# DanEngelbrecht/longtail

Measured on AMD Instinct MI355X. Metric: ingest GB/s (chunk+hash+compress), higher is better.
Workload: dtype u8/u32

## Files before the change

longtail_amd/csrc/k_buzhash.hip:

```cpp
#include "lthip_internal.h"

#include <stdlib.h>
#include <type_traits>

namespace
{

__constant__ uint32_t c_buztab[256] = {
#include "buzhash_table.inc"
};

constexpr int RUN = 64;
constexpr int TILE = 256 * RUN;
constexpr int ROW_DW = 17;
constexpr int TAB_REP = 64;

__device__ __forceinline__ uint32_t lds_load_u32(uint32_t byte_addr)
{
#if defined(__HIP_DEVICE_COMPILE__)
    return *(const __attribute__((address_space(3))) uint32_t*)byte_addr;
#else
    (void)byte_addr;
    return 0u;
#endif
// ... 139 lines not shown
    auto group = [&](auto G) __attribute__((always_inline))
    {
        constexpr int g = decltype(G)::value;
        uint32_t y[8];
#pragma unroll
        for (int half = 1; half >= 0; --half)
        {
            if (half == 1)
                halo_wait(std::integral_constant<int, 2 * g + 1 + 4>{});
            else
                halo_wait(std::integral_constant<int, 2 * g + 4>{});
#pragma unroll
            for (int ii = 3; ii >= 0; --ii)
            {
                const int i = 4 * half + ii;
                const int k = 8 * g + i;
                uint32_t w;
                if (k >= 47)
                    w = S[k - 47] ^ S[k + 1];
                else
                    w = (S[0] ^ S[k + 1]) ^ (uint32_t)__builtin_amdgcn_update_dpp(0, (int)S[(k + 17) & 63], 0x13C, 0xf, 0xf, false);
                const uint32_t h = (k & 31) ? rotl32(w, (uint32_t)(k & 31)) : w;
                if (MODE == 1)
                    y[i] = ~h & (dv.d - 1u);
                else
                {
#if K1_MAD64
                    uint64_t t, carry;
                    asm("v_mad_u64_u32 %0, %1, %2, %3, %4" : "=v"(t), "=s"(carry) : "v"(h), "s"(dv.inv), "v"(inv64));
                    y[i] = (uint32_t)t;
#else
                    y[i] = h * dv.inv + inv_v;
#endif
                }
            }
            if (half == 1)
                halo_quad(std::integral_constant<int, 2 * g + 2>{});
            else
                halo_quad(std::integral_constant<int, 2 * g + 1>{});
        }
        const uint32_t m = min(min(min(y[0], y[1]), y[2]), min(min(min(y[3], y[4]), y[5]), min(y[6], y[7])));
        if (__builtin_amdgcn_ballot_w64(m <= pc.thr) != 0ull)
        {
            asm volatile("");
#pragma unroll
            for (int i = 0; i < 8; ++i)
            {
                const int k = 8 * g + i;
                if (__builtin_amdgcn_ballot_w64(y[i] <= pc.thr) != 0ull)
                {
                    asm volatile("");
                    const bool hit = MODE == 1 ? y[i] == 0u : rotr32(y[i] + pc.exact_add, dv.k2) <= dv.qlim;
                    uint32_t hbit;
                    asm volatile("v_cndmask_b32_e64 %0, 0, 1, %1" : "=v"(hbit) : "s"(__builtin_amdgcn_ballot_w64(hit)));
                    if (k < 32)
                        mlo |= hbit << k;
                    else
                        mhi |= hbit << (k - 32);
                }
            }
        }
    };
    group(std::integral_constant<int, 7>{});
    group(std::integral_constant<int, 6>{});
    group(std::integral_constant<int, 5>{});
    group(std::integral_constant<int, 4>{});
    group(std::integral_constant<int, 3>{});
    group(std::integral_constant<int, 2>{});
    group(std::integral_constant<int, 1>{});
    group(std::integral_constant<int, 0>{});
    return ((uint64_t)mhi << 32) | mlo;
}

__device__ __forceinline__ uint64_t prefix_legal(uint64_t m, uint64_t q0, uint64_t size)
{
    if (q0 >= size)
        return 0ull;
    if (q0 < 47)
        m &= ~0ull << (47 - q0);
    const uint64_t remain = size - q0;
    if (remain < 64)
        m &= (1ull << remain) - 1ull;
    return m;
}

__device__ __forceinline__ void prefix_table_init(uint32_t* tab, int tid, int nthreads)
{
    for (int v = tid; v < 256; v += nthreads)
    {
        const uint32_t tv = c_buztab[v];
        uint4 q = make_uint4(tv, tv, tv, tv);
        uint4* dst = reinterpret_cast<uint4*>(tab + v * TAB_REP);
#pragma unroll
        for (int j = 0; j < TAB_REP / 4; ++j)
            dst[j] = q;
    }
    __syncthreads();
    if ((uint32_t)(uintptr_t)(const __attribute__((address_space(3))) uint32_t*)tab != 0u)
        __builtin_trap();
}

#ifdef LTHIP_ABLATIONS
#include "ablations/k_buzhash_prefix_regs.inc"
#endif

constexpr int DMA_BUF_B = WROWS * 64;

struct TileDma
{
    const uint8_t* data;
    uint32_t* buf;
    int lane;
    uint32_t buf_byte;
    uint32_t buf_mid;
    uint32_t src_off;
    uint32_t own_row;
    uint32_t own_f;

    __device__ __forceinline__ TileDma(const uint8_t* d, uint32_t* b, int ln) : data(d), buf(b), lane(ln)
    {
        buf_byte = __builtin_amdgcn_readfirstlane((uint32_t)(uintptr_t)(const __attribute__((address_space(3))) uint32_t*)buf);
        buf_mid = buf_byte + 2048u;
        const uint32_t src_vec = 4u * ((uint32_t)lane >> 2) + (((uint32_t)lane & 3u) ^ (((uint32_t)lane >> 4) & 3u));
        src_off = 16u * src_vec;
        own_f = (((uint32_t)lane + 1u) >> 2) & 3u;
        own_row = buf_byte + 64u * ((uint32_t)lane + 1u);
    }

    template <int MODE>
    __device__ __forceinline__ PrefixConsts consts(const DivTest& dv) const
    {
        PrefixConsts pc;
        pc.lane4 = (uint32_t)lane * 4u;
        pc.hj = 63u - (uint32_t)lane;
        pc.halo_byte = buf_byte + DMA_BUF_B;
        pc.thr = MODE == 1 ? 0u : 0xFFFFFFFFu / (dv.d >> dv.k2);
        pc.exact_add = dv.addc - dv.inv;
        return pc;
    }

    template <int u>
    __device__ __forceinline__ void piece(const uint8_t* mid_src) const
    {
        asm volatile("s_mov_b32 m0, %[l]\n\ts_nop 0\n\t"
                     "global_load_lds_dwordx4 %[v], %[b] offset:%[o]"
                     :
                     : [v] "v"(src_off), [l] "s"(buf_mid), [b] "s"(mid_src), [o] "i"(1024 * u - 2048)
                     : "memory");
    }

    template <int u>
    __device__ __forceinline__ void edge(const PartDev& p, uint64_t sp, const uint8_t* mid_src) const
    {
        const int64_t g = (int64_t)sp - 64 + 1024 * u + (int64_t)src_off;
        const bool lane_on = u < 4 || lane < 4;
        const bool whole = lane_on && g >= 0 && (uint64_t)g + 16 <= p.size;
        const bool part = lane_on && g >= 0 && (uint64_t)g < p.size && (uint64_t)g + 16 > p.size;
        if (whole)
            piece<u>(mid_src);
        if (part)
        {
            const uint8_t* src = data + p.off;
            uint32_t w[4] = {0, 0, 0, 0};
            const uint32_t n = (uint32_t)(p.size - (uint64_t)g);
            for (uint32_t bb = 0; bb < n; ++bb)
                w[bb >> 2] |= (uint32_t)src[g + bb] << (8 * (bb & 3));
            uint32_t* d = buf + 256 * u + 4 * lane;
            d[0] = w[0];
            d[1] = w[1];
            d[2] = w[2];
            d[3] = w[3];
        }
    }

    __device__ __forceinline__ void issue(const PartDev& p, uint64_t sp) const
    {
        const uint8_t* mid_src = data + p.off + sp - 64 + 2048;
        if (sp >= 64 && sp + (uint64_t)WTILE <= p.size)
        {
            asm volatile("s_mov_b32 m0, %[l]\n\ts_nop 0\n\t"
                         "global_load_lds_dwordx4 %[v], %[b] offset:-2048\n\t"
                         "global_load_lds_dwordx4 %[v], %[b] offset:-1024\n\t"
                         "global_load_lds_dwordx4 %[v], %[b] offset:0\n\t"
                         "global_load_lds_dwordx4 %[v], %[b] offset:1024"
                         :
                         : [v] "v"(src_off), [l] "s"(buf_mid), [b] "s"(mid_src)
                         : "memory");
            if (lane < 4)
                piece<4>(mid_src);
        }
        else
        {
            edge<0>(p, sp, mid_src);
            edge<1>(p, sp, mid_src);
            edge<2>(p, sp, mid_src);
            edge<3>(p, sp, mid_src);
            edge<4>(p, sp, mid_src);
        }
    }

    __device__ __forceinline__ void take(uint32_t (&win)[16], uint32_t& hb, const PrefixConsts& pc) const
    {
        asm volatile("s_waitcnt vmcnt(0)" ::: "memory");
#pragma unroll
        for (int c = 0; c < 4; ++c)
        {
            const uint4 q = lds_load_u128(own_row + 16u * ((uint32_t)c ^ own_f));
            win[4 * c + 0] = q.x;
            win[4 * c + 1] = q.y;
            win[4 * c + 2] = q.z;
            win[4 * c + 3] = q.w;
        }
        hb = lds_load_u8(buf_byte + pc.hj);
        asm volatile("s_waitcnt lgkmcnt(0)" ::: "memory");
    }
};

template <int MODE, int WAVES>
__global__ __launch_bounds__(64 * WAVES, 1) void k_buzhash_prefix_dma(const uint8_t* __restrict__ data,
                                                                       const PartDev* __restrict__ parts,
                                                                       const uint32_t* __restrict__ tile_part,
                                                                       uint32_t ntiles, DivTest dv,
                                                                       uint64_t* __restrict__ bm0,
                                                                       uint64_t* __restrict__ bm1)
{
    extern __shared__ __attribute__((aligned(16))) uint32_t smem[];
    const int tid = threadIdx.x;
    const int lane = tid & 63;
    const int wave = __builtin_amdgcn_readfirstlane(tid >> 6);
    uint32_t* buf = smem + 256 * TAB_REP + wave * ((DMA_BUF_B >> 2) + HALO_DW);
    uint32_t* halo = buf + (DMA_BUF_B >> 2);
    prefix_table_init(smem, tid, 64 * WAVES);

    const TileDma dma(data, buf, lane);
    const PrefixConsts pc = dma.consts<MODE>(dv);

    const uint64_t nwt = (uint64_t)ntiles * 4u;
    const uint64_t wstride = (uint64_t)gridDim.x * (uint64_t)WAVES;
    uint64_t wt = (uint64_t)blockIdx.x * (uint64_t)WAVES + (uint64_t)wave;
    if (wt >= nwt)
        return;

    PartDev pd = parts[tile_part[wt >> 2]];
    uint64_t span = ((wt >> 2) - pd.tile_base) * (uint64_t)TILE + (wt & 3u) * (uint64_t)WTILE;
    dma.issue(pd, span);

    uint64_t pend_m = 0, pend_summary = 0, pend_i0 = 0, pend_i1 = 0;
    bool pend = false;
    for (;;)
    {
        uint32_t win[16], hb;
        dma.take(win, hb, pc);

        if (pend)
        {
            if (pend_m != 0ull)
                bm0[pend_i0 + (uint64_t)lane] = pend_m;
            if (lane == 0)
                bm1[pend_i1] = pend_summary;
        }

        const uint64_t next = wt + wstride;
        PartDev npd = pd;
        uint64_t next_span = 0;
        if (next < nwt)
        {
            npd = parts[tile_part[next >> 2]];
            next_span = ((next >> 2) - npd.tile_base) * (uint64_t)TILE + (next & 3u) * (uint64_t)WTILE;
            dma.issue(npd, next_span);
        }

        pend_m = prefix_legal(prefix_tile<MODE>(win, hb, pc, dv, lane, halo), span + (uint64_t)lane * RUN, pd.size);
        pend_summary = __builtin_amdgcn_ballot_w64(pend_m != 0ull);
        pend_i0 = pd.bm0_base + (span >> 6);
        pend_i1 = pd.bm1_base + (span >> 12);
        pend = true;

        if (next >= nwt)
            break;
        wt = next;
        pd = npd;
        span = next_span;
    }
    if (pend_m != 0ull)
        bm0[pend_i0 + (uint64_t)lane] = pend_m;
    if (lane == 0)
        bm1[pend_i1] = pend_summary;
}

__device__ __forceinline__ uint64_t bcast64(uint64_t v, int src_lane)
{
    uint32_t lo = __builtin_amdgcn_readlane((uint32_t)v, src_lane);
    uint32_t hi = __builtin_amdgcn_readlane((uint32_t)(v >> 32), src_lane);
    return ((uint64_t)hi << 32) | lo;
}

__global__ __launch_bounds__(64) void k_select_cuts(const PartDev* __restrict__ parts, uint32_t nparts,
                                                    const uint64_t* __restrict__ bm0, const uint64_t* __restrict__ bm1,
                                                    uint32_t min_chunk, uint32_t max_chunk, uint2* __restrict__ region,
                                                    uint32_t* __restrict__ part_count)
{
    const uint32_t p = blockIdx.x;
    if (p >= nparts)
        return;
    const int lane = threadIdx.x;
    const PartDev pd = parts[p];
    const uint64_t size = pd.size;
    const uint64_t* b0 = bm0 + pd.bm0_base;
    const uint64_t* b1 = bm1 + pd.bm1_base;
    uint2* out = region + pd.region_base;

    uint64_t s = 0;
    uint32_t n = 0;
    while (s < size)
    {
        const uint64_t left = size - s;
        uint64_t len;
        if (left <= min_chunk)
            len = left;
        else
        {
            const uint64_t end = left > max_chunk ? max_chunk : left;
            len = end;
            const uint64_t qlo = s + min_chunk;
            const uint64_t qhi = s + end - 1;
            if (qlo <= qhi)
            {
                const uint64_t rlo = qlo >> 6, rhi = qhi >> 6;
                const uint64_t wlo = rlo >> 6, whi = rhi >> 6;
                bool found = false;
                for (uint64_t w0 = wlo; w0 <= whi && !found; w0 += 64)
                {
                    const uint64_t w = w0 + (uint64_t)lane;
                    uint64_t word = 0;
                    if (w <= whi)
                    {
                        word = b1[w];
                        if (w == wlo)
                            word &= ~0ull << (rlo & 63);
                        if (w == whi && (rhi & 63) != 63)
                            word &= (1ull << ((rhi & 63) + 1)) - 1ull;
                    }
                    for (;;)
                    {
                        const uint64_t any = __builtin_amdgcn_ballot_w64(word != 0ull);
                        if (any == 0ull)
                            break;
                        const int f = __builtin_ctzll(any);
                        const uint64_t fw = bcast64(word, f);
                        const int bit = __builtin_ctzll(fw);
                        const uint64_t r = ((w0 + (uint64_t)f) << 6) + (uint64_t)bit;
                        uint64_t m = b0[r];
                        if (r == rlo)
                            m &= ~0ull << (qlo & 63);
                        if (r == rhi && (qhi & 63) != 63)
                            m &= (1ull << ((qhi & 63) + 1)) - 1ull;
                        if (m != 0ull)
                        {
                            const uint64_t q = (r << 6) + (uint64_t)__builtin_ctzll(m);
                            len = q - s + 1;
                            found = true;
                            break;
                        }
                        if (lane == f)
                            word &= word - 1ull;
                    }
                }
            }
        }
        if (lane == 0)
            out[n] = make_uint2((uint32_t)s, (uint32_t)len);
        ++n;
        s += len;
    }
    if (lane == 0)
        part_count[p] = n;
}

#ifdef LTHIP_ABLATIONS
__device__ unsigned long long g_walk_tiles;
#endif

template <int MODE, int WAVES, bool GUESS>
__global__ __launch_bounds__(64 * WAVES, 1) void k_buzhash_walk(const uint8_t* __restrict__ data, const PartDev* __restrict__ parts,
                                                                 uint32_t nparts, DivTest dv, uint32_t min_chunk, uint32_t max_chunk,
                                                                 uint2* __restrict__ region, uint32_t* __restrict__ part_count,
                                                                 uint32_t* __restrict__ ticket)
{
    extern __shared__ __attribute__((aligned(16))) uint32_t smem[];
    const int tid = threadIdx.x;
    const int lane = tid & 63;
    const int wave = __builtin_amdgcn_readfirstlane(tid >> 6);
    uint32_t* buf = smem + 256 * TAB_REP + wave * ((DMA_BUF_B >> 2) + HALO_DW);
    uint32_t* halo = buf + (DMA_BUF_B >> 2);
    prefix_table_init(smem, tid, 64 * WAVES);

    const TileDma dma(data, buf, lane);
    const PrefixConsts pc = dma.consts<MODE>(dv);
    const int lane_base = lane * RUN;

    auto jump = [](uint64_t q) __attribute__((always_inline)) { return q >= 64 ? ((q - 64) & ~(uint64_t)15) + 64 : (uint64_t)0; };

    bool inflight = false;
    uint64_t inflight_tb = 0;
#ifdef LTHIP_ABLATIONS
    uint32_t tiles = 0;
#endif
    for (;;)
    {
        __builtin_amdgcn_wave_barrier();
        uint32_t t = atomicAdd(ticket, lane == 0 ? 1u : 0u);
        t = __builtin_amdgcn_readfirstlane(t);
        if (t >= nparts)
            break;
        const PartDev pd = parts[t];
        const uint64_t size = pd.size;
        uint2* out = region + pd.region_base;
        uint64_t s = 0, qlo = 0, qhi = 0;
        uint32_t n = 0, end = 0;

        auto next_chunk = [&]() __attribute__((always_inline)) -> bool
        {
            for (;;)
            {
                if (s >= size)
                    return false;
                const uint64_t left = size - s;
                const uint32_t len = left <= min_chunk ? (uint32_t)left : left > max_chunk ? max_chunk : (uint32_t)left;
                if (left > min_chunk && len > min_chunk)
                {
                    end = len;
                    qlo = s + min_chunk;
                    qhi = s + end - 1;
                    return true;
                }
                if (lane == 0)
                    out[n] = make_uint2((uint32_t)s, len);
                ++n;
                s += len;
            }
        };

        if (next_chunk())
        {
            uint64_t tb = jump(qlo);
            for (bool walking = true; walking;)
            {
                if (!(inflight && inflight_tb == tb))
                {
                    if (inflight)
                        asm volatile("s_waitcnt vmcnt(0)" ::: "memory");
                    dma.issue(pd, tb);
                }
                inflight = false;
                uint32_t win[16], hb;
                dma.take(win, hb, pc);
                if (GUESS)
                {
                    uint64_t g = tb + (uint64_t)WTILE;
                    bool aim = true;
                    if (g > qhi)
                    {
                        const uint64_t s2 = s + end;
                        aim = size - s2 > min_chunk && max_chunk > min_chunk;
                        g = jump(s2 + min_chunk);
                    }
                    if (aim)
                    {
                        dma.issue(pd, g);
                        inflight = true;
                        inflight_tb = g;
                    }
                }
                const uint64_t raw = prefix_tile<MODE>(win, hb, pc, dv, lane, halo);
#ifdef LTHIP_ABLATIONS
                ++tiles;
#endif
                for (;;)
                {
                    const int lo = (int)(qlo > tb ? qlo - tb : 0) - lane_base;
                    const int hi = (int)(qhi - tb < (uint64_t)WTILE ? qhi - tb : (uint64_t)WTILE - 1) - lane_base;
                    uint64_t m = raw;
                    if (lo > 0)
                        m = lo > 63 ? 0ull : m & (~0ull << lo);
                    if (hi < 63)
                        m = hi < 0 ? 0ull : m & ((2ull << hi) - 1ull);
                    const uint64_t any = __builtin_amdgcn_ballot_w64(m != 0ull);
                    uint32_t len;
                    if (any != 0ull)
                    {
                        const int f = __builtin_ctzll(any);
                        const uint64_t q = tb + (uint64_t)(f * RUN + __builtin_ctzll(bcast64(m, f)));
                        len = (uint32_t)(q - s) + 1u;
                    }
                    else if (qhi - tb < (uint64_t)WTILE)
                        len = end;
                    else
                    {
                        tb += (uint64_t)WTILE;
                        break;
                    }
                    if (lane == 0)
                        out[n] = make_uint2((uint32_t)s, len);
                    ++n;
                    s += len;
                    if (!next_chunk())
                    {
                        walking = false;
                        break;
                    }
                    if (qlo >= tb && qlo - tb < (uint64_t)WTILE)
                        continue;
                    tb = jump(qlo);
                    break;
                }
            }
        }
        if (inflight)
        {
            asm volatile("s_waitcnt vmcnt(0)" ::: "memory");
            inflight = false;
        }
        if (lane == 0)
            part_count[t] = n;
    }
#ifdef LTHIP_ABLATIONS
    if (lane == 0 && tiles)
        atomicAdd(&g_walk_tiles, (unsigned long long)tiles);
#endif
}

constexpr int SCAN_THREADS = 256;
constexpr int SCAN_ITEMS = 8;
constexpr int SCAN_BLOCK = SCAN_THREADS * SCAN_ITEMS;

__device__ __forceinline__ uint32_t block_exclusive_scan(uint32_t v, uint32_t* total, uint32_t* sh )
{
    const int lane = threadIdx.x & 63, wave = threadIdx.x >> 6;
    uint32_t x = v;
#pragma unroll
    for (int o = 1; o < 64; o <<= 1)
    {
        uint32_t y = __shfl_up(x, o, 64);
        if (lane >= o)
            x += y;
    }
    if (lane == 63)
        sh[wave] = x;
    __syncthreads();
    uint32_t base = 0, tot = 0;
#pragma unroll
    for (int w = 0; w < SCAN_THREADS / 64; ++w)
    {
        uint32_t t = sh[w];
        if (w < wave)
            base += t;
        tot += t;
    }
    __syncthreads();
    *total = tot;
    return base + x - v;
}

__global__ __launch_bounds__(SCAN_THREADS) void k_scan_sums(const uint32_t* __restrict__ in, uint64_t n,
                                                            const uint32_t* __restrict__ n_dev,
                                                            uint32_t* __restrict__ sums)
{
    __shared__ uint32_t sh[8];
    if (n_dev)
        n = *n_dev < n ? *n_dev : n;
    const uint64_t base = (uint64_t)blockIdx.x * SCAN_BLOCK;
    uint32_t acc = 0;
#pragma unroll
    for (int i = 0; i < SCAN_ITEMS; ++i)
    {
        uint64_t idx = base + (uint64_t)i * SCAN_THREADS + threadIdx.x;
        if (idx < n)
            acc += in[idx];
    }
    uint32_t tot;
    block_exclusive_scan(acc, &tot, sh);
    if (threadIdx.x == 0)
        sums[blockIdx.x] = tot;
}

__global__ __launch_bounds__(SCAN_THREADS) void k_scan_spine(uint32_t* __restrict__ sums, uint32_t nblocks)
{
    __shared__ uint32_t sh[8];
    uint32_t carry = 0;
    for (uint32_t b0 = 0; b0 < nblocks; b0 += SCAN_THREADS)
    {
        uint32_t i = b0 + threadIdx.x;
        uint32_t v = i < nblocks ? sums[i] : 0;
        uint32_t tot;
        uint32_t ex = block_exclusive_scan(v, &tot, sh);
        if (i < nblocks)
            sums[i] = carry + ex;
        carry += tot;
    }
    if (threadIdx.x == 0)
        sums[nblocks] = carry;
}

__global__ __launch_bounds__(SCAN_THREADS) void k_scan_apply(const uint32_t* __restrict__ in, uint64_t n,
                                                             const uint32_t* __restrict__ n_dev,
                                                             const uint32_t* __restrict__ sums, uint32_t nblocks,
                                                             uint32_t* __restrict__ out)
{
    __shared__ uint32_t sh[8];
    if (n_dev)
        n = *n_dev < n ? *n_dev : n;
    const uint64_t base = (uint64_t)blockIdx.x * SCAN_BLOCK + (uint64_t)threadIdx.x * SCAN_ITEMS;
    uint32_t v[SCAN_ITEMS];
    uint32_t acc = 0;
#pragma unroll
    for (int i = 0; i < SCAN_ITEMS; ++i)
    {
        uint64_t idx = base + i;
        v[i] = idx < n ? in[idx] : 0;
        acc += v[i];
    }
    uint32_t tot;
    uint32_t ex = block_exclusive_scan(acc, &tot, sh) + sums[blockIdx.x];
#pragma unroll
    for (int i = 0; i < SCAN_ITEMS; ++i)
    {
        uint64_t idx = base + i;
        if (idx < n)
            out[idx] = ex;
        ex += v[i];
    }
    if (blockIdx.x == 0 && threadIdx.x == 0)
        out[n] = sums[nblocks];
}

__global__ __launch_bounds__(64) void k_compact_chunks(const PartDev* __restrict__ parts, uint32_t nparts,
                                                       const uint2* __restrict__ region,
                                                       const uint32_t* __restrict__ part_first,
                                                       uint64_t* __restrict__ chunk_offsets,
                                                       uint32_t* __restrict__ chunk_lens)
{
    const uint32_t p = blockIdx.x;
    if (p >= nparts)
        return;
    const PartDev pd = parts[p];
    const uint32_t first = part_first[p];
    const uint32_t n = part_first[p + 1] - first;
    const uint2* in = region + pd.region_base;
    for (uint32_t i = threadIdx.x; i < n; i += 64)
    {
        uint2 e = in[i];
        chunk_offsets[first + i] = pd.off + (uint64_t)e.x;
        chunk_lens[first + i] = e.y;
    }
}

__global__ __launch_bounds__(64) void k_chunk_from_buffer(const uint8_t* __restrict__ buf, uint32_t n, uint32_t min_chunk,
                                                          DivTest dv, uint64_t* __restrict__ out_len)
{
    const int lane = threadIdx.x;
    uint32_t h0 = 0;
    for (uint32_t i = 0; i < 48; ++i)
        h0 ^= rotl32(c_buztab[buf[i]], (47u - i) & 31u);
    uint32_t result = n;
// ... 278 lines not shown
```

longtail_amd/csrc/lthip_ctx.hip:

```cpp
#include "lthip_internal.h"

#include <stdlib.h>

int lthip_fail(lthip_ctx* ctx, int code, const char* what, const char* detail)
{
    if (ctx)
        snprintf(ctx->err, sizeof ctx->err, "%s: %s", what ? what : "?", detail ? detail : "");
    return code;
}

int lthip_scratch(lthip_ctx* ctx, int slot, size_t bytes, void** out)
{
    if (bytes == 0)
        bytes = 256;
    if (ctx->scratch_cap[slot] < bytes)
    {
        if (ctx->scratch[slot])
        {
            LTHIP_CHECK(ctx, lthip_stream_wait(ctx));
            LTHIP_CHECK(ctx, hipFree(ctx->scratch[slot]));
            ctx->scratch[slot] = nullptr;
            ctx->scratch_cap[slot] = 0;
        }
        size_t cap = bytes + bytes / 8 + 4096;
// ... 509 lines not shown
    block_starts[nb] = i;
    *out_block_count = nb;
    *out_next_chunk = i;
    return 0;
}

extern "C" int lthip_divtest_eval(uint32_t discriminator, uint32_t hash)
{
    if (discriminator == 0)
        return 0;
    const DivTest t = make_div_test(discriminator);
    if (t.pow2)
        return (hash & (t.d - 1u)) == t.d - 1u;
    const uint32_t m = hash * t.inv + t.addc;
    const uint32_t r = t.k2 ? ((m >> t.k2) | (m << (32u - t.k2))) : m;
    return r <= t.qlim;
}

static uint32_t plan_slice_points(uint32_t part_count, const uint64_t* part_sizes, uint32_t want, uint32_t* first)
{
    if (part_count < 2 || want < 2)
        return 0;
    uint64_t total = 0;
    for (uint32_t p = 0; p < part_count; ++p)
        total += part_sizes[p];
    if (total < LTHIP_SLICE_MIN_BYTES)
        return 0;
    uint32_t S = want > part_count ? part_count : want;
    while (S > 2 && total / S < LTHIP_SLICE_MIN_BYTES / 2)
        --S;
    uint64_t acc = 0;
    uint32_t p = 0;
    first[0] = 0;
    for (uint32_t k = 1; k < S; ++k)
    {
        const uint64_t goal = total / S * k;
        while (p < part_count - (S - k) && acc + part_sizes[p] / 2 < goal)
            acc += part_sizes[p++];
        if (p <= first[k - 1])
        {
            acc += part_sizes[p];
            ++p;
        }
        first[k] = p;
    }
    first[S] = part_count;
    return S;
}

static int plan_layout(lthip_ctx* ctx, const char* what, uint32_t min_chunk, uint32_t part_count, const uint64_t* part_offsets,
                       const uint64_t* part_sizes, PartDev* parts, PlanExtents& x)
{
    memset(&x, 0, sizeof x);
    x.nparts = part_count;
    for (uint32_t p = 0; p < part_count; ++p)
    {
        const uint64_t sz = part_sizes[p];
        if ((part_offsets[p] & 15u) != 0 || sz > 0xFFFFFFFFull)
            return lthip_fail(ctx, EINVAL, what, "part offsets must be 16-byte aligned, sizes < 4 GiB");
        PartDev& pd = parts[p];
        memset(&pd, 0, sizeof pd);
        pd.off = part_offsets[p];
        pd.size = sz;
        pd.bm0_base = x.bm0_words;
        pd.bm1_base = x.bm1_words;
        pd.region_base = x.chunk_cap;
        pd.tile_base = (uint32_t)x.ntiles;
        const uint64_t cap = sz ? sz / min_chunk + 1 : 0;
        pd.region_cap = (uint32_t)cap;
        const uint64_t t = div_up_u64(sz, 16384);
        x.ntiles += t;
        x.bm0_words += t * 256;
        x.bm1_words += t * 4;
        x.chunk_cap += cap;
        x.total_bytes += sz;
        x.leaf_cap += div_up_u64(sz, 1024) + cap;
        x.nonempty_parts += sz != 0;
        x.max_part_bytes = sz > x.max_part_bytes ? sz : x.max_part_bytes;
    }
    return 0;
}

static bool plan_walk_rule(const lthip_plan* plan)
{
    const uint64_t waves = lthip_k1_resident_waves(plan->device);
    return plan->nonempty_parts >= LTHIP_WALK_MIN_PARTS_PER_WAVE * waves &&
           plan->max_part_bytes * LTHIP_WALK_MAX_PART_DIV <= plan->total_bytes / waves;
}

static int plan_create_impl(lthip_ctx* ctx, uint32_t part_count, const uint64_t* part_offsets, const uint64_t* part_sizes,
                            uint32_t min_chunk, uint32_t avg_chunk, uint32_t max_chunk, lthip_plan** out_plan)
{
    if (!ctx || !out_plan || (part_count && (!part_offsets || !part_sizes)))
        return EINVAL;
    *out_plan = nullptr;
    if (min_chunk < 48 || min_chunk > avg_chunk || avg_chunk > max_chunk)
        return lthip_fail(ctx, EINVAL, "lthip_plan_create", "need 48 <= min <= avg <= max");
    uint32_t d = discriminator_from_avg(avg_chunk);
    if (d == 0)
        return lthip_fail(ctx, EINVAL, "lthip_plan_create", "discriminator is zero");
    LTHIP_CHECK(ctx, hipSetDevice(ctx->device));
    std::vector<PartDev> parts(part_count);
    PlanExtents x;
    int err = plan_layout(ctx, "lthip_plan_create", min_chunk, part_count, part_offsets, part_sizes, parts.data(), x);
    if (err)
        return err;
    if (x.ntiles > 0xFFFFFFF0ull)
        return lthip_fail(ctx, EINVAL, "lthip_plan_create", "batch too large");

    lthip_plan* plan = new (std::nothrow) lthip_plan();
    if (!plan)
        return ENOMEM;
    memset(plan, 0, sizeof *plan);
    static_cast<PlanExtents&>(*plan) = x;
    plan->device = ctx->device;
    plan->min_chunk = min_chunk;
    plan->avg_chunk = avg_chunk;
    plan->max_chunk = max_chunk;
    plan->div = make_div_test(d);
    plan->capacity_bytes = x.total_bytes;
    plan->cap_parts = part_count ? part_count : 1;
    plan->cap_tiles = x.ntiles ? x.ntiles : 1;
    plan->walked = plan_walk_rule(plan);

    hipError_t e = lthip_hip_malloc((void**)&plan->d_parts, sizeof(PartDev) * plan->cap_parts);
    if (e == hipSuccess)
        e = lthip_hip_malloc((void**)&plan->d_tile_part, sizeof(uint32_t) * plan->cap_tiles);
    if (e == hipSuccess && part_count)
        e = hipMemcpyAsync(plan->d_parts, parts.data(), sizeof(PartDev) * part_count, hipMemcpyHostToDevice, ctx->stream);
    if (e == hipSuccess)
        e = lthip_stream_wait(ctx);
    if (e != hipSuccess)
    {
        lthip_plan_destroy(ctx, plan);
        return lthip_fail(ctx, e == hipErrorOutOfMemory ? ENOMEM : EIO, "lthip_plan_create", hipGetErrorString(e));
    }
    if ((err = lthip_launch_tile_table(ctx, plan)))
    {
        lthip_plan_destroy(ctx, plan);
        return err;
    }
    *out_plan = plan;
    return 0;
}

static int plan_aim(lthip_ctx* ctx, lthip_plan* plan, const PlanExtents& x, const PartDev* parts)
{
    static_cast<PlanExtents&>(*plan) = x;
    plan->walked = plan_walk_rule(plan);
    const int err = lthip_stage_upload(ctx, plan->d_parts, parts, sizeof(PartDev) * x.nparts, ctx->stream);
    return err ? err : lthip_launch_tile_table(ctx, plan);
}

static void plan_aim_slices(lthip_ctx* ctx, lthip_plan* plan, uint32_t want, const uint64_t* part_offsets, const uint64_t* part_sizes)
{
    plan->sliced = false;
    uint32_t first[9];
    const uint32_t S = plan_slice_points(plan->nparts, part_sizes, want, first);
    if (S == 0 || (plan->nslices && S != plan->nslices))
        return;
    bool ok = true;
    if (!plan->nslices)
        for (uint32_t k = 0; k < S && ok; ++k)
            ok = plan_create_impl(ctx, first[k + 1] - first[k], part_offsets + first[k], part_sizes + first[k], plan->min_chunk,
                                  plan->avg_chunk, plan->max_chunk, &plan->slice[k]) == 0;
    else
    {
        std::vector<PartDev> parts(plan->nparts);
        PlanExtents x[8];
        for (uint32_t k = 0; k < S && ok; ++k)
        {
            const uint32_t n = first[k + 1] - first[k];
            ok = plan_layout(ctx, "lthip_plan_reaim", plan->min_chunk, n, part_offsets + first[k], part_sizes + first[k], &parts[first[k]],
                             x[k]) == 0 &&
                 n <= plan->slice[k]->cap_parts && x[k].ntiles <= plan->slice[k]->cap_tiles;
        }
        for (uint32_t k = 0; k < S && ok; ++k)
            ok = plan_aim(ctx, plan->slice[k], x[k], &parts[first[k]]) == 0;
    }
    if (!ok)
    {
        if (!plan->nslices)
            for (uint32_t k = 0; k < S; ++k)
            {
                lthip_plan_destroy(ctx, plan->slice[k]);
                plan->slice[k] = nullptr;
            }
        ctx->err[0] = 0;
        return;
    }
    memcpy(plan->slice_first, first, sizeof(uint32_t) * (S + 1));
    plan->nslices = S;
    plan->sliced = true;
}

extern "C" int lthip_plan_create(lthip_ctx* ctx, uint32_t part_count, const uint64_t* part_offsets,
                                 const uint64_t* part_sizes, uint32_t min_chunk, uint32_t avg_chunk, uint32_t max_chunk,
                                 lthip_plan** out_plan)
{
    int err = plan_create_impl(ctx, part_count, part_offsets, part_sizes, min_chunk, avg_chunk, max_chunk, out_plan);
    if (err)
        return err;
    int want = LTHIP_SLICES;
    LTHIP_ABLATION_ENV(env_slices, "LTHIP_SLICES");
    if (env_slices.get() > 0)
        want = env_slices.get() > 8 ? 8 : env_slices.get();
    plan_aim_slices(ctx, *out_plan, (uint32_t)want, part_offsets, part_sizes);
    return 0;
}

extern "C" int lthip_plan_resize_single(lthip_ctx* ctx, lthip_plan* plan, uint64_t size)
{
    if (!ctx || !plan || plan->nparts != 1)
        return EINVAL;
    if (size > plan->capacity_bytes)
        return lthip_fail(ctx, EINVAL, "lthip_plan_resize_single", "size above the capacity the plan was created with");
    LTHIP_CHECK(ctx, hipSetDevice(ctx->device));
    const uint64_t off = 0;
    PartDev pd;
    PlanExtents x;
    const int err = plan_layout(ctx, "lthip_plan_resize_single", plan->min_chunk, 1, &off, &size, &pd, x);
    if (err)
        return err;
    static_cast<PlanExtents&>(*plan) = x;
    return lthip_stage_upload(ctx, plan->d_parts, &pd, sizeof pd, ctx->stream);
}

extern "C" int lthip_plan_reaim(lthip_ctx* ctx, lthip_plan* plan, uint32_t part_count, const uint64_t* part_offsets,
                                const uint64_t* part_sizes)
{
    if (!ctx || !plan || (part_count && (!part_offsets || !part_sizes)))
        return EINVAL;
    if (part_count == 0 || part_count > plan->cap_parts)
        return lthip_fail(ctx, EINVAL, "lthip_plan_reaim", "part count outside 1 .. the count the plan was created with");
    LTHIP_CHECK(ctx, hipSetDevice(ctx->device));
    {
        std::vector<PartDev> parts(part_count);
        PlanExtents x;
        int err = plan_layout(ctx, "lthip_plan_reaim", plan->min_chunk, part_count, part_offsets, part_sizes, parts.data(), x);
        if (err)
            return err;
        if (x.ntiles > plan->cap_tiles)
            return lthip_fail(ctx, EINVAL, "lthip_plan_reaim", "more 16 KiB tiles than the plan was created with");
        if ((err = plan_aim(ctx, plan, x, parts.data())))
            return err;
    }
    if (plan->nslices)
        plan_aim_slices(ctx, plan, plan->nslices, part_offsets, part_sizes);
    return 0;
}

extern "C" void lthip_plan_destroy(lthip_ctx* ctx, lthip_plan* plan)
{
    if (!plan)
        return;
    (void)hipSetDevice(plan->device);
    if (ctx)
        (void)lthip_stream_wait(ctx);
    else
        (void)hipDeviceSynchronize();
    if (plan->d_parts)
        (void)hipFree(plan->d_parts);
    if (plan->d_tile_part)
        (void)hipFree(plan->d_tile_part);
    for (uint32_t k = 0; k < 8; ++k)
        lthip_plan_destroy(ctx, plan->slice[k]);
    delete plan;
}

extern "C" uint64_t lthip_plan_chunk_capacity(const lthip_plan* plan) { return plan ? plan->chunk_cap : 0; }
extern "C" uint32_t lthip_plan_slices(const lthip_plan* plan) { return plan && plan->sliced ? plan->nslices : 1u; }

static bool plan_walks(const lthip_plan* plan)
{
    LTHIP_ABLATION_ENV(env_walk, "LTHIP_K1_WALK");
    if (env_walk.get() >= 0)
        return env_walk.get() != 0 && plan->nparts != 0;
    return plan->walked;
}
extern "C" uint32_t lthip_plan_walked_scans(const lthip_plan* plan)
{
    if (!plan)
        return 0;
    if (!plan->sliced)
        return plan_walks(plan);
    uint32_t n = 0;
    for (uint32_t k = 0; k < plan->nslices; ++k)
        n += plan_walks(plan->slice[k]);
    return n;
}

struct ScanBuffers
{
    uint64_t *bm0, *bm1;
    uint2* region;
    uint32_t* part_count;
};
static int chunk_scan_buffers(lthip_ctx* ctx, const lthip_plan* plan, bool bitmaps, ScanBuffers* b)
{
    b->bm0 = b->bm1 = nullptr;
    int err;
    if (bitmaps && ((err = lthip_scratch(ctx, S_BM0, plan->bm0_words * 8, (void**)&b->bm0)) ||
                    (err = lthip_scratch(ctx, S_BM1, plan->bm1_words * 8, (void**)&b->bm1))))
        return err;
    if ((err = lthip_scratch(ctx, S_REGION, plan->chunk_cap * sizeof(uint2), (void**)&b->region)))
        return err;
    return lthip_scratch(ctx, S_PART_COUNT, ((size_t)plan->nparts + 1) * 4, (void**)&b->part_count);
}

static int chunk_scan(lthip_ctx* ctx, const lthip_plan* plan, const void* d_data, const ScanBuffers& b)
{
    if (!plan->nparts)
        return 0;
    return plan_walks(plan) ? lthip_launch_buzhash_walk(ctx, plan, (const uint8_t*)d_data, b.region, b.part_count)
                            : lthip_launch_buzhash(ctx, plan, (const uint8_t*)d_data, b.bm0, b.bm1);
}

static int chunk_cut_hash(lthip_ctx* ctx, const lthip_plan* plan, const void* d_data, const ScanBuffers& b, uint64_t* d_offsets,
                          uint32_t* d_lens, uint64_t* d_hashes, uint32_t* d_part_first)
{
    int err;
    if (plan->nparts && !plan_walks(plan) && (err = lthip_launch_select(ctx, plan, b.bm0, b.bm1, b.region, b.part_count)))
        return err;
    if ((err = lthip_launch_compact(ctx, plan, b.region, b.part_count, d_part_first, d_offsets, d_lens)))
        return err;
    return d_hashes ? lthip_launch_blake3(ctx, (const uint8_t*)d_data, d_offsets, d_lens, d_part_first + plan->nparts, plan->chunk_cap,
                                          plan->leaf_cap, plan->max_chunk, d_hashes)
                    : 0;
}

__global__ void k_slice_join(const uint64_t* __restrict__ b_off, const uint32_t* __restrict__ b_len, const uint64_t* __restrict__ b_hash,
                             const uint32_t* __restrict__ b_first, uint32_t nparts_b, uint32_t* __restrict__ part_first ,
                             uint64_t* __restrict__ offs, uint32_t* __restrict__ lens, uint64_t* __restrict__ hashes)
{
    const uint32_t base = part_first[0], total_b = b_first[nparts_b];
    const uint64_t i = (uint64_t)blockIdx.x * blockDim.x + threadIdx.x;
    if (i < total_b)
    {
        offs[base + i] = b_off[i];
        lens[base + i] = b_len[i];
        hashes[base + i] = b_hash[i];
    }
    if (i >= 1 && i <= nparts_b)
        part_first[i] = b_first[i] + base;
}

// ... 141 lines not shown
```

Baseline: 903.4.

## Simplify edge/bound arithmetic to 32-bit and skip slicing for walking plans

Edge handling in the buzhash DMA tile loader now computes the valid byte window per 1 KiB piece with 32-bit comparisons. It reads partial tails relative to the mid source pointer instead of doing 64-bit per-lane bounds checks. The bitmap store base is forced into scalar registers, and the cut-walk range tests use unsigned 32-bit wraparound compares. On the host, plans that use the walk rule no longer run in sliced mode unless LTHIP_SLICES is set, which changes how the pipeline schedules slices.

```diff
diff --git a/longtail_amd/csrc/k_buzhash.hip b/longtail_amd/csrc/k_buzhash.hip
--- a/longtail_amd/csrc/k_buzhash.hip
+++ b/longtail_amd/csrc/k_buzhash.hip
@@ -315,19 +315,24 @@
     template <int u>
     __device__ __forceinline__ void edge(const PartDev& p, uint64_t sp, const uint8_t* mid_src) const
     {
-        const int64_t g = (int64_t)sp - 64 + 1024 * u + (int64_t)src_off;
-        const bool lane_on = u < 4 || lane < 4;
-        const bool whole = lane_on && g >= 0 && (uint64_t)g + 16 <= p.size;
-        const bool part = lane_on && g >= 0 && (uint64_t)g < p.size && (uint64_t)g + 16 > p.size;
+        const int64_t base = (int64_t)sp - 64 + 1024 * u;
+        const int64_t left = (int64_t)p.size - base;
+        const int32_t left_hi = (int32_t)(left >> 32);
+        const uint32_t before = base < 0 ? (uint32_t)-base : 0u;
+        const uint32_t room = left_hi < 0 ? 0u : left_hi > 0 || (uint32_t)left > 1024u ? 1024u : (uint32_t)left;
+        const uint32_t room16 = room & ~15u;
+        const bool lane_on = (u < 4 || lane < 4) && src_off >= before;
+        const bool whole = lane_on && src_off < room16;
+        const bool part = lane_on && src_off == room16 && room != room16;
         if (whole)
             piece<u>(mid_src);
         if (part)
         {
-            const uint8_t* src = data + p.off;
+            const uint8_t* src = mid_src + (1024 * u - 2048);
             uint32_t w[4] = {0, 0, 0, 0};
-            const uint32_t n = (uint32_t)(p.size - (uint64_t)g);
+            const uint32_t n = room - src_off;
             for (uint32_t bb = 0; bb < n; ++bb)
-                w[bb >> 2] |= (uint32_t)src[g + bb] << (8 * (bb & 3));
+                w[bb >> 2] |= (uint32_t)src[src_off + bb] << (8 * (bb & 3));
             uint32_t* d = buf + 256 * u + 4 * lane;
             d[0] = w[0];
             d[1] = w[1];
@@ -379,6 +384,13 @@
     }
 };
 
+__device__ __forceinline__ uint64_t* run_words(uint64_t* __restrict__ bm0, uint64_t first)
+{
+    uint64_t* w = bm0 + first;
+    asm("" : "+s"(w));
+    return w;
+}
+
 template <int MODE, int WAVES>
 __global__ __launch_bounds__(64 * WAVES, 1) void k_buzhash_prefix_dma(const uint8_t* __restrict__ data,
                                                                        const PartDev* __restrict__ parts,
@@ -418,7 +430,7 @@
         if (pend)
         {
             if (pend_m != 0ull)
-                bm0[pend_i0 + (uint64_t)lane] = pend_m;
+                run_words(bm0, pend_i0)[(uint32_t)lane] = pend_m;
             if (lane == 0)
                 bm1[pend_i1] = pend_summary;
         }
@@ -426,7 +438,8 @@
         const uint64_t next = wt + wstride;
         PartDev npd = pd;
         uint64_t next_span = 0;
-        if (next < nwt)
+        const bool more = (int64_t)(next - nwt) < 0;
+        if (more)
         {
             npd = parts[tile_part[next >> 2]];
             next_span = ((next >> 2) - npd.tile_base) * (uint64_t)TILE + (next & 3u) * (uint64_t)WTILE;
@@ -439,14 +452,14 @@
         pend_i1 = pd.bm1_base + (span >> 12);
         pend = true;
 
-        if (next >= nwt)
+        if (!more)
             break;
         wt = next;
         pd = npd;
         span = next_span;
     }
     if (pend_m != 0ull)
-        bm0[pend_i0 + (uint64_t)lane] = pend_m;
+        run_words(bm0, pend_i0)[(uint32_t)lane] = pend_m;
     if (lane == 0)
         bm1[pend_i1] = pend_summary;
 }
@@ -607,6 +620,7 @@
         if (next_chunk())
         {
             uint64_t tb = jump(qlo);
+            auto ends_here = [&]() __attribute__((always_inline)) { return (uint32_t)(qhi - tb) < (uint32_t)WTILE; };
             for (bool walking = true; walking;)
             {
                 if (!(inflight && inflight_tb == tb))
@@ -622,7 +636,7 @@
                 {
                     uint64_t g = tb + (uint64_t)WTILE;
                     bool aim = true;
-                    if (g > qhi)
+                    if (ends_here())
                     {
                         const uint64_t s2 = s + end;
                         aim = size - s2 > min_chunk && max_chunk > min_chunk;
@@ -642,7 +656,7 @@
                 for (;;)
                 {
                     const int lo = (int)(qlo > tb ? qlo - tb : 0) - lane_base;
-                    const int hi = (int)(qhi - tb < (uint64_t)WTILE ? qhi - tb : (uint64_t)WTILE - 1) - lane_base;
+                    const int hi = (int)(ends_here() ? (uint32_t)(qhi - tb) : (uint32_t)WTILE - 1u) - lane_base;
                     uint64_t m = raw;
                     if (lo > 0)
                         m = lo > 63 ? 0ull : m & (~0ull << lo);
@@ -656,7 +670,7 @@
                         const uint64_t q = tb + (uint64_t)(f * RUN + __builtin_ctzll(bcast64(m, f)));
                         len = (uint32_t)(q - s) + 1u;
                     }
-                    else if (qhi - tb < (uint64_t)WTILE)
+                    else if (ends_here())
                         len = end;
                     else
                     {
@@ -672,7 +686,7 @@
                         walking = false;
                         break;
                     }
-                    if (qlo >= tb && qlo - tb < (uint64_t)WTILE)
+                    if ((uint32_t)(qlo - tb) < (uint32_t)WTILE)
                         continue;
                     tb = jump(qlo);
                     break;
diff --git a/longtail_amd/csrc/lthip_ctx.hip b/longtail_amd/csrc/lthip_ctx.hip
--- a/longtail_amd/csrc/lthip_ctx.hip
+++ b/longtail_amd/csrc/lthip_ctx.hip
@@ -685,9 +685,14 @@
     return err ? err : lthip_launch_tile_table(ctx, plan);
 }
 
+static bool plan_walks(const lthip_plan* plan);
 static void plan_aim_slices(lthip_ctx* ctx, lthip_plan* plan, uint32_t want, const uint64_t* part_offsets, const uint64_t* part_sizes)
 {
     plan->sliced = false;
+    LTHIP_ABLATION_ENV(env_slices, "LTHIP_SLICES");
+    const bool as_one = plan_walks(plan) && env_slices.get() <= 0;
+    if (as_one && plan->nslices)
+        return;
     uint32_t first[9];
     const uint32_t S = plan_slice_points(plan->nparts, part_sizes, want, first);
     if (S == 0 || (plan->nslices && S != plan->nslices))
@@ -724,7 +729,7 @@
     }
     memcpy(plan->slice_first, first, sizeof(uint32_t) * (S + 1));
     plan->nslices = S;
-    plan->sliced = true;
+    plan->sliced = !as_one;
 }
 
 extern "C" int lthip_plan_create(lthip_ctx* ctx, uint32_t part_count, const uint64_t* part_offsets,
```

New measurement: 913.4, median of 6. 1.01x the previous value.
